# unslothai/unsloth

Hardware: AMD Instinct MI355X
Metric: train tokens/sec, Llama-3-8B QLoRA (NF4) r=16 seq2048 bf16 (higher is better)
Workload: dtype bf16; 1 GPU; Llama-3-8B QLoRA NF4 r=16 (q,k,v,o,gate,up,down) seq2048 bf16, fwd+bwd+AdamW; model=Llama-3-8B (synthetic weights), global_batch=4, seq_len=2048, parallelism=dp1, layers=32, lora_rank=16, gradient_checkpointing=unsloth, gc_schedule_chosen=all (every layer keeps everything), nf4_decoded_weight_mirrors=off (every NF4 weight is decoded at every use INSIDE the timed step), trainable_params=41943040, attention=csrc/attention.hip (causal GQA flash, fwd+bwd), optimizer=FlatAdamW fp32 on LoRA params

## Files before the change

include/unsloth_amd.h:

```cpp
#ifndef UNSLOTH_AMD_H
#define UNSLOTH_AMD_H

#include <stdint.h>

#ifdef __cplusplus
extern "C" {
#endif

#define UAMD_OK 0
#define UAMD_ERR_DTYPE (-1)
#define UAMD_ERR_ARG (-2)
#define UAMD_ERR_ALIGN (-3)

#define UAMD_F32 0
#define UAMD_F16 1
#define UAMD_BF16 2

int uamd_version(void);

int uamd_rms_layernorm_fwd(const void* X, const void* W, void* Y, float* r, int64_t n_rows,
                           int n_cols, int64_t x_row_stride, int64_t y_row_stride, float eps,
                           int gemma, int x_dtype, int w_dtype, void* stream);
int uamd_rms_layernorm_bwd(const void* dY, void* dX, const void* X, const void* W, const float* r,
                           int64_t n_rows, int n_cols, int64_t dy_row_stride,
// ... 124 lines not shown
int uamd_gemm_tn_256(const void* A, int64_t lda, int M, int K, const uamd_gemm_group* groups,
                     int n_groups, int accumulate, int dtype, void* stream);
#define UAMD_TUNE_GLU_VAR 0
#define UAMD_TUNE_GROUP_M 1
#define UAMD_TUNE_STREAM_NT 2
#define UAMD_TUNE_DEQUANT_T 3
#define UAMD_TUNE_ATTN_VAR 4
#define UAMD_TUNE_RMS_VAR 5
#define UAMD_TUNE_GEMM_HALF 6
#define UAMD_TUNE_GEMM_PERSIST 7
#define UAMD_TUNE_DEQUANT_X4 8
#define UAMD_TUNE_GEMM_PLAIN 9
#define UAMD_TUNE_GLU_XA 10
#define UAMD_TUNE_GEMM_S 11
#define UAMD_TUNE_COUNT 12
int uamd_set_tuning(int knob, int value);
int uamd_gemm_nt_nf4(const void* A, int64_t lda, int M, int K, const uamd_gemm_group* groups,
                     int n_groups, int accumulate, int dtype, void* stream);
int uamd_lora_xa(const void* X, int64_t ldx, const void* A, int64_t lda, float* out,
                 int64_t ld_out, int M, int K, int R, int out_cols, int dtype, void* stream);

typedef struct {
    const float* P;
    const void* Z;
    float* out;
    int64_t ldp, ldz, ldo;
    int N;
    int R;
    int out_nr;
    float scale;
} uamd_lora_tn_problem;
int uamd_lora_tn(const uamd_lora_tn_problem* probs, int n_probs, int M, float* workspace,
                 int64_t workspace_floats, int dtype, void* stream);

int uamd_attn_fwd(const void* Q, const void* K, const void* V, void* O, float* LSE, const int64_t* strides,
                  int B, int T, int Hq, int Hk, int D, int lse_stride, float scale, int causal, const int* lo,
                  int dtype, void* stream);
int uamd_attn_bwd(const void* Q, const void* K, const void* V, const void* O, const void* dO, const float* LSE,
                  void* dQ, void* dK, void* dV, float* Delta, const int64_t* strides, int B, int T, int Hq, int Hk,
                  int D, int lse_stride, float scale, int causal, const int* lo, const int* hi, int dtype,
                  void* stream);
int uamd_attn_fwd_band(const void* Q, const void* K, const void* V, void* O, float* LSE, const int64_t* strides,
                       int B, int T, int Hq, int Hk, int D, int lse_stride, float scale, int causal, const int* lo,
                       const int* hi, int dtype, void* stream);

typedef struct {
    const void* W;
    const uint8_t* absmax_u8;
    const float* absmax_f32;
    const float* code2;
    const float* absmax2;
    void* y;
    const float* lora_t;
    const void* lora_b;
    const void* bias;
    int64_t ldw, ld_lb;
    float offset, lora_scale;
    int N, R, blocksize2, lora_b_f32, y_f32, _pad;
} uamd_gemv_group;
int uamd_gemv(const void* x, int K, const uamd_gemv_group* groups, int n_groups, int nf4, int blocksize, int dtype,
              void* stream);
#define UAMD_GEMV_SYNC_BYTES (8 * 256)
#define UAMD_TAG_STRIDE 1024u
typedef struct {
    int mode, Rt, w_f32, glu;
    const void* x2;
// ... 61 lines not shown
```

unsloth_amd/_lib.py:

```python
import ctypes
import os
from contextlib import nullcontext

import torch

c_void_p, c_int, c_int64, c_float = ctypes.c_void_p, ctypes.c_int, ctypes.c_int64, ctypes.c_float

HERE = os.path.dirname(os.path.abspath(__file__))
LIB_PATH = os.environ.get("UNSLOTH_AMD_LIB") or os.path.join(HERE, "lib", "libunsloth_amd.so")

UAMD_F32, UAMD_F16, UAMD_BF16 = 0, 1, 2
_DTYPE_CODE = {torch.float32: UAMD_F32, torch.float16: UAMD_F16, torch.bfloat16: UAMD_BF16}
_ERR = {-1: "unsupported dtype", -2: "invalid argument", -3: "pointer/stride not 16-byte aligned"}


class GemmGroup(ctypes.Structure):

    _fields_ = [
        ("B", c_void_p), ("C", c_void_p), ("absmax", c_void_p), ("lora_xa", c_void_p),
        ("lora_b", c_void_p), ("ldb", c_int64), ("ldc", c_int64), ("ld_xa", c_int64),
        ("ld_lb", c_int64), ("N", c_int), ("R", c_int), ("lora_scale", c_float), ("_pad", c_int),
        ("lora_xk", c_void_p), ("lora_bk", c_void_p), ("ld_xk", c_int64), ("ld_bk", c_int64), ("Rk", c_int),
        ("_pad2", c_int), ("bias", c_void_p),
    ]
# ... 77 lines not shown
    "uamd_gemm_nn_256": (c_int, [c_void_p, c_int64, c_int, c_int, ctypes.POINTER(GemmGroup), c_int, c_int,
                                 c_int, c_void_p]),
    "uamd_gemm_tn_256": (c_int, [c_void_p, c_int64, c_int, c_int, ctypes.POINTER(GemmGroup), c_int, c_int,
                                 c_int, c_void_p]),
    "uamd_set_tuning": (c_int, [c_int, c_int]),
    "uamd_gemm_nt_nf4": (c_int, [c_void_p, c_int64, c_int, c_int, ctypes.POINTER(GemmGroup), c_int,
                                 c_int, c_int, c_void_p]),
    "uamd_lora_xa": (c_int, [c_void_p, c_int64, c_void_p, c_int64, c_void_p, c_int64, c_int, c_int,
                             c_int, c_int, c_int, c_void_p]),
    "uamd_lora_xa2": (c_int, [c_void_p, c_int64, c_void_p, c_int64, c_void_p, c_int64, c_int, c_int,
                              c_int, c_int, c_int, c_void_p]),
    "uamd_lora_xa2k": (c_int, [c_void_p, c_int64, c_void_p, c_int64, c_void_p, c_int64, c_void_p, c_int64, c_int,
                               c_int, c_int, c_int, c_int, c_int, c_void_p]),
    "uamd_add_rms_layernorm_fwd": (c_int, [c_void_p] * 6 + [c_int64, c_int, c_int64, c_int64, c_int64, c_int64, c_float,
                                                             c_int, c_int, c_void_p]),
    "uamd_add_rms_layernorm_bwd": (c_int, [c_void_p] * 6 + [c_int64, c_int, c_int64, c_int64, c_int64, c_int64, c_int,
                                                             c_int, c_void_p]),
    "uamd_lora_prepare": (c_int, [c_void_p, c_void_p, c_int, c_int, c_int, c_void_p]),
    "uamd_adamw_flat": (c_int, [c_void_p, c_void_p, c_void_p, c_void_p, c_int64] + [ctypes.c_double] * 8 + [c_int, c_void_p]),
    "uamd_glu_fwd_xa": (c_int, [c_int, c_void_p, c_void_p, c_void_p, c_int, c_int, c_int64, c_void_p, c_int64, c_int,
                                c_void_p, c_int64, c_int, c_void_p, c_int64, c_int, c_int, c_void_p]),
    "uamd_glu_bwd_xa": (c_int, [c_int, c_void_p, c_void_p, c_void_p, c_int, c_int, c_int64]
                        + [c_void_p, c_int64, c_int, c_void_p, c_int64, c_int, c_void_p, c_int64, c_int] * 2
                        + [c_int, c_void_p]),
    "uamd_glu_xa_workspace": (c_int64, [c_int, c_int, c_int, c_int]),
    "uamd_glu_fwd_xa_ws": (c_int, [c_int, c_void_p, c_void_p, c_void_p, c_int, c_int, c_int64, c_void_p, c_int64, c_int,
                                   c_void_p, c_int64, c_int, c_void_p, c_int64, c_int, c_void_p, c_int64, c_void_p, c_int, c_void_p]),
    "uamd_glu_bwd_xa_ws": (c_int, [c_int, c_void_p, c_void_p, c_void_p, c_int, c_int, c_int64]
                           + [c_void_p, c_int64, c_int, c_void_p, c_int64, c_int, c_void_p, c_int64, c_int] * 2
                           + [c_void_p, c_int64, c_void_p, c_int, c_void_p]),
    "uamd_adamw_shard": (c_int, [c_void_p, c_void_p, c_void_p, c_void_p, c_void_p, c_int64] + [ctypes.c_double] * 8
                         + [c_int, c_void_p]),
    "uamd_lora_tn": (c_int, [ctypes.POINTER(LoraTnProblem), c_int, c_int, c_void_p, c_int64, c_int, c_void_p]),
    "uamd_attn_fwd": (c_int, [c_void_p, c_void_p, c_void_p, c_void_p, c_void_p, ctypes.POINTER(c_int64), c_int, c_int,
                              c_int, c_int, c_int, c_int, c_float, c_int, c_void_p, c_int, c_void_p]),
    "uamd_attn_fwd_band": (c_int, [c_void_p, c_void_p, c_void_p, c_void_p, c_void_p, ctypes.POINTER(c_int64), c_int, c_int,
                                   c_int, c_int, c_int, c_int, c_float, c_int, c_void_p, c_void_p, c_int, c_void_p]),
    "uamd_attn_bwd": (c_int, [c_void_p] * 10 + [ctypes.POINTER(c_int64), c_int, c_int, c_int, c_int, c_int, c_int,
                                               c_float, c_int, c_void_p, c_void_p, c_int, c_void_p]),
    "uamd_gemv": (c_int, [c_void_p, c_int, ctypes.POINTER(GemvGroup), c_int, c_int, c_int, c_int, c_void_p]),
    "uamd_gemv_fused": (c_int, [c_void_p, c_int, ctypes.POINTER(GemvGroup), c_int, c_int, c_int, c_int, c_void_p,
                                ctypes.POINTER(GemvPrologue)]),
    "uamd_rope_kv_append": (c_int, [c_void_p, c_int64, c_void_p, c_void_p, c_int64, c_void_p, c_void_p, c_void_p, c_void_p,
                                    c_int64, c_int64, c_int, c_int, c_int, c_int, c_int, c_int, c_void_p]),
    "uamd_attn_decode": (c_int, [c_void_p, c_int64, c_void_p, c_void_p, c_int64, c_int64, c_void_p, c_int, c_void_p,
                                 c_void_p, c_int64, c_int, c_int, c_int, c_int, c_int, c_int, c_int, c_float, c_int,
                                 c_void_p]),
    "uamd_attn_decode_fused": (c_int, [c_void_p, c_int64, c_void_p, c_void_p, c_int64, c_void_p, c_void_p, c_void_p, c_void_p,
                                       c_int64, c_int64, c_void_p, c_void_p, c_void_p, c_int64, c_int, c_int, c_int, c_int,
                                       c_int, c_int, c_int, c_int, c_float, ctypes.c_uint, c_void_p, c_int, c_void_p]),
    "uamd_argmax_f32": (c_int, [c_void_p, c_int, c_int64, c_void_p, c_void_p, c_void_p, c_void_p]),
    "uamd_debug_mfma_probe": (c_int, [c_void_p, c_void_p]),
}

_LIB = None


def lib():
    global _LIB
    if _LIB is None:
        if not os.path.exists(LIB_PATH):
            raise RuntimeError(
                f"unsloth_amd: {LIB_PATH} is missing. Build it with `python -m unsloth_amd._build` "
                "(hipcc, gfx950). There is no CPU / PyTorch fallback for the fused kernels."
            )
        handle = ctypes.CDLL(LIB_PATH)
# ... 47 lines not shown
```

unsloth_amd/csrc/glu.hip:

```cpp
#include "common.h"

namespace {

enum { ACT_SWIGLU = 0, ACT_GEGLU_EXACT = 1, ACT_GEGLU_APPROX = 2 };
#ifndef UAMD_GLU_KNOCK
#define UAMD_GLU_KNOCK 0
#endif

__device__ __forceinline__ float sigmoidf_(float x) { return uamd_sigmoid(x); }

template <int ACT>
__device__ __forceinline__ void act_fwd(float e, float& f) {
    if (ACT == ACT_SWIGLU) {
        f = e * sigmoidf_(e);
    } else if (ACT == ACT_GEGLU_EXACT) {
        f = 0.5f * e * (erff(0.70710678118654752440f * e) + 1.0f);
    } else {
        const float s = 0.7978845608028654f;
        f = 0.5f * e * (tanhf(s * e * (1.0f + 0.044715f * e * e)) + 1.0f);
    }
}

template <int ACT>
__device__ __forceinline__ void act_bwd(float e, float& f, float& dfde) {
// ... 539 lines not shown
    return UAMD_OK;
}

int64_t xa_ws_floats(int M, int K, int NS, int R) {
    const int NT = R <= 16 ? 1 : (R <= 32 ? 2 : 4);
    const int ntiles = (K + GX_TK - 1) / GX_TK;
    return (int64_t)((M + 15) / 16) * ((ntiles + GX_TPB - 1) / GX_TPB) * 16 * (NS * NT * 16);
}

template <int NS>
int glu_xa_entry(int act, void* dw, void* e, void* g, void* h, int M, int K, int64_t ld, const GluXaOut& o0,
                 const GluXaOut& o1, int dtype, void* stream, float* ws = nullptr, int64_t ws_floats = 0, int* counters = nullptr) {
    if (M < 0 || K <= 0 || !e || !g || (NS == 1 ? !h : !dw)) return UAMD_ERR_ARG;
    if (M == 0) return UAMD_OK;
    if ((K & 7) || (ld & 7) || !aligned16(e) || !aligned16(g) || (NS == 1 ? !aligned16(h) : !aligned16(dw))) return UAMD_ERR_ALIGN;
    int rc = check_xa_out(o0, K);
    if (rc) return rc;
    if (NS > 1 && (rc = check_xa_out(o1, K))) return rc;
    hipStream_t st = (hipStream_t)stream;
    if (ws != nullptr && ws_floats < xa_ws_floats(M, K, NS, NS > 1 ? (o0.R > o1.R ? o0.R : o1.R) : o0.R)) return UAMD_ERR_ARG;
#define GLU_XA_CASE(TT, DC)                                                                          \
    if (dtype == DC) {                                                                              \
        if (act == ACT_SWIGLU) return launch_xa<TT, ACT_SWIGLU, NS>(dw, e, g, h, M, K, ld, o0, o1, st, ws, counters);          \
        if (act == ACT_GEGLU_EXACT) return launch_xa<TT, ACT_GEGLU_EXACT, NS>(dw, e, g, h, M, K, ld, o0, o1, st, ws, counters); \
        if (act == ACT_GEGLU_APPROX) return launch_xa<TT, ACT_GEGLU_APPROX, NS>(dw, e, g, h, M, K, ld, o0, o1, st, ws, counters); \
        return UAMD_ERR_ARG;                                                                        \
    }
    GLU_XA_CASE(bf16_t, UAMD_BF16)
    GLU_XA_CASE(f16_t, UAMD_F16)
#undef GLU_XA_CASE
    return UAMD_ERR_DTYPE;
}

}

extern "C" int uamd_glu_fwd_xa(int act, const void* e, const void* g, void* h, int M, int K, int64_t ld, const void* W,
                               int64_t ldw, int R, float* out, int64_t ld_out, int out_cols, void* out_k, int64_t ld_k,
                               int k_cols, int dtype, void* stream) {
    GluXaOut o0{out, ld_out, R, out_cols, out_k, ld_k, k_cols, W, ldw};
    return glu_xa_entry<1>(act, nullptr, const_cast<void*>(e), const_cast<void*>(g), h, M, K, ld, o0, o0, dtype, stream);
}

extern "C" int uamd_glu_bwd_xa(int act, void* DW, void* e, void* g, int M, int K, int64_t ld,
                               const void* Wu, int64_t ldwu, int Ru, float* out_u, int64_t ld_out_u, int out_cols_u,
                               void* out_k_u, int64_t ld_k_u, int k_cols_u,
                               const void* Wg, int64_t ldwg, int Rg, float* out_g, int64_t ld_out_g, int out_cols_g,
                               void* out_k_g, int64_t ld_k_g, int k_cols_g, int dtype, void* stream) {
    GluXaOut o0{out_u, ld_out_u, Ru, out_cols_u, out_k_u, ld_k_u, k_cols_u, Wu, ldwu};
    GluXaOut o1{out_g, ld_out_g, Rg, out_cols_g, out_k_g, ld_k_g, k_cols_g, Wg, ldwg};
    return glu_xa_entry<2>(act, DW, e, g, nullptr, M, K, ld, o0, o1, dtype, stream);
}

extern "C" int64_t uamd_glu_xa_workspace(int M, int K, int n_products, int max_rank) {
    if (M < 0 || K <= 0 || n_products < 1 || n_products > 2 || max_rank < 1 || max_rank > 64) return -1;
    return xa_ws_floats(M, K, n_products, max_rank);
}
extern "C" int uamd_glu_fwd_xa_ws(int act, const void* e, const void* g, void* h, int M, int K, int64_t ld, const void* W,
                                  int64_t ldw, int R, float* out, int64_t ld_out, int out_cols, void* out_k, int64_t ld_k,
                                  int k_cols, float* ws, int64_t ws_floats, int* counters, int dtype, void* stream) {
    GluXaOut o0{out, ld_out, R, out_cols, out_k, ld_k, k_cols, W, ldw};
    return glu_xa_entry<1>(act, nullptr, const_cast<void*>(e), const_cast<void*>(g), h, M, K, ld, o0, o0, dtype, stream, ws,
                           ws_floats, counters);
}
extern "C" int uamd_glu_bwd_xa_ws(int act, void* DW, void* e, void* g, int M, int K, int64_t ld,
                                  const void* Wu, int64_t ldwu, int Ru, float* out_u, int64_t ld_out_u, int out_cols_u,
                                  void* out_k_u, int64_t ld_k_u, int k_cols_u,
                                  const void* Wg, int64_t ldwg, int Rg, float* out_g, int64_t ld_out_g, int out_cols_g,
                                  void* out_k_g, int64_t ld_k_g, int k_cols_g, float* ws, int64_t ws_floats, int* counters,
                                  int dtype, void* stream) {
    GluXaOut o0{out_u, ld_out_u, Ru, out_cols_u, out_k_u, ld_k_u, k_cols_u, Wu, ldwu};
    GluXaOut o1{out_g, ld_out_g, Rg, out_cols_g, out_k_g, ld_k_g, k_cols_g, Wg, ldwg};
    return glu_xa_entry<2>(act, DW, e, g, nullptr, M, K, ld, o0, o1, dtype, stream, ws, ws_floats, counters);
}

namespace {
template <typename T, bool BWD>
__global__ void __launch_bounds__(256) quick_gelu_kernel(const T* __restrict__ X, T* __restrict__ Y, int64_t n) {
    constexpr int VEC = Vec16<T>::N;
    const int64_t nvec = n / VEC;
    for (int64_t i = (int64_t)blockIdx.x * 256 + threadIdx.x; i < nvec; i += (int64_t)gridDim.x * 256) {
        Vec16<T> x = ld16_m(X + i * VEC, 0), y;
        if (BWD) y = ld16_m(Y + i * VEC, 0);
#pragma unroll
        for (int j = 0; j < VEC; ++j) {
            const float v = to_f32(x.e[j]);
            const float sg = uamd_sigmoid(1.702f * v);
            if (BWD) y.e[j] = from_f32<T>(to_f32(y.e[j]) * (sg + 1.702f * v * sg * (1.0f - sg)));
            else y.e[j] = from_f32<T>(v * sg);
        }
        st16_m(Y + i * VEC, y, 0);
    }
    if (blockIdx.x == 0) {
        for (int64_t k = nvec * VEC + threadIdx.x; k < n; k += 256) {
            const float v = to_f32(X[k]);
            const float sg = uamd_sigmoid(1.702f * v);
            Y[k] = from_f32<T>(BWD ? to_f32(Y[k]) * (sg + 1.702f * v * sg * (1.0f - sg)) : v * sg);
        }
    }
}
template <typename T, bool BWD>
int launch_quick_gelu(const void* x, void* y, int64_t n, hipStream_t st) {
    if (!aligned16(x) || !aligned16(y)) return UAMD_ERR_ALIGN;
    const int64_t nvec = n / Vec16<T>::N;
    int64_t blocks = (nvec + 255) / 256;
    if (blocks < 1) blocks = 1;
    if (blocks > 256 * 16) blocks = 256 * 16;
    hipLaunchKernelGGL((quick_gelu_kernel<T, BWD>), dim3((unsigned)blocks), dim3(256), 0, st, (const T*)x, (T*)y, n);
// ... 36 lines not shown
```

unsloth_amd/kernels/fast_lora.py:

```python
import os

import torch

from .utils import _same_rows, alloc_rows, glu_bwd_terms, glu_fwd_xa
from .utils import (
    GRAD_SINKS,
    grad_sink,
    cast_lora,
    get_lora_parameters,
    lora_dx_terms,
    lora_linear_dx,
    lora_linear_forward,
    lora_tn,
    lora_tn_supported,
)
from .swiglu import swiglu_fg_kernel, swiglu_DWf_DW_dfg_kernel
from .geglu import (
    geglu_exact_forward_kernel,
    geglu_exact_backward_kernel,
    geglu_approx_forward_kernel,
    geglu_approx_backward_kernel,
)

try:
# ... 7 lines not shown
def _lora_grads(X2d, dY2d, A, B, s, dtype):
    if A is None:
        return None, None
    At, Bt = cast_lora(A, dtype).t(), cast_lora(B, dtype).t()
    dA_t = torch.empty_like(At)
    dB_t = torch.empty_like(Bt)
    dA_t.addmm_(X2d.t(), dY2d @ Bt.t(), alpha=s, beta=0)
    dB_t.addmm_(At.t() @ X2d.t(), dY2d, alpha=s, beta=0)
    return dA_t.t(), dB_t.t()


def _lora_grads_fused(items):
    probs, slots, targets, sinks = [], [], [], []
    for (X2d, dY2d, A, B, s, XA, P) in items:
        if A is None:
            slots.append(None)
            continue
        r = A.shape[0]
        slots.append(len(probs))
        probs.append((P, X2d, r, False, s))
        probs.append((XA, dY2d, r, True, s))
        for prm in (A, B):
            sink = grad_sink(prm)
            sinks.append((sink, prm))
            targets.append(sink.grad_view(prm) if sink is not None else None)
    outs = lora_tn(probs, targets if any(t is not None for t in targets) else None)
    for sink, prm in sinks:
        if sink is not None:
            sink.ready(prm)
    outs = [None if sk[0] is not None else o for o, sk in zip(outs, sinks)]
    return [(None, None) if k is None else (outs[k], outs[k + 1]) for k in slots]


_ACT_NAMES = {swiglu_fg_kernel: "swiglu", swiglu_DWf_DW_dfg_kernel: "swiglu",
              geglu_exact_forward_kernel: "geglu_exact", geglu_exact_backward_kernel: "geglu_exact",
              geglu_approx_forward_kernel: "geglu_approx", geglu_approx_backward_kernel: "geglu_approx"}


MERGE_GATE_UP = True


def _gate_up(X, gate, up, return_xa=False):
    outs = None
    widths = [(q.shape[0] if q is not None else W.shape[0]) for (W, q, *_rest) in (gate, up)]
    if (MERGE_GATE_UP and X.is_cuda and X.dtype in (torch.bfloat16, torch.float16) and widths[0] == widths[1]
            and widths[0] % 64 == 0 and all(len(p) <= 5 or p[5] is None for p in (gate, up))):
        M = X.numel() // X.shape[-1]
        eg = alloc_rows(M, 2 * widths[0], X.dtype, X.device)
        outs = [eg[:, :widths[0]], eg[:, widths[0]:]]
    return lora_linear_forward(X, [gate, up], outs=outs, return_xa=return_xa)


def mlp_forward(X, gate, up, down, act_fwd):
    (e, g), xa_gu = _gate_up(X, gate, up, return_xa=True)
    act = _ACT_NAMES.get(act_fwd)
    e2, g2 = e.view(-1, e.shape[-1]), g.view(-1, g.shape[-1])
    fused = glu_fwd_xa(act, e2, g2, down) if (act is not None and _same_rows([e2, g2])) else None
    if fused is not None:
        h, pre = fused
        (out,), xa_d = lora_linear_forward(h.view(e.shape), [down], return_xa=True, pre_xa=pre)
    else:
        if not e.is_contiguous():
            e, g = e.contiguous(), g.contiguous()
        h = act_fwd(e, g)
        (out,), xa_d = lora_linear_forward(h, [down], return_xa=True)
    return out, e, g, (xa_gu[0], xa_gu[1], xa_d[0])


def mlp_gate_up_forward(X, gate, up):
    return _gate_up(X, gate, up)


def mlp_backward(dY, X, e, g, xas, gate, up, down, act_bwd, inplace=True):
    xa_g, xa_u, xa_d = xas
    shape = X.shape
    dY = dY.reshape(-1, dY.shape[-1])
    X2 = X.reshape(-1, X.shape[-1])
    e = e.view(-1, e.shape[-1])
    g = g.view(-1, g.shape[-1])
    dtype = X2.dtype
    (p_d,) = lora_dx_terms([dY], [down])
    padded = e.stride(0) != e.shape[1] and _same_rows([e, g])
    DW = lora_linear_dx([dY], [down], terms=[p_d],
                        out=alloc_rows(e.shape[0], e.shape[1], e.dtype, e.device, ld=e.stride(0)) if padded else None)
    act = _ACT_NAMES.get(act_bwd)
    fused = glu_bwd_terms(act, DW, e, g, up, gate) if (act is not None and DW.dim() == 2) else None
    if fused is not None:
        h, df, de, (p_u, p_g) = fused
    else:
        if padded:
            DW, e, g = DW.contiguous(), e.contiguous(), g.contiguous()
        DW, e, g = act_bwd(DW, e, g)
        h, df, de = DW, e, g
        p_u, p_g = lora_dx_terms([df, de], [up, gate])
    if lora_tn_supported([h, dY, X2, df, de]):
        (d_downA, d_downB), (d_upA, d_upB), (d_gateA, d_gateB) = _lora_grads_fused([
            (h, dY, down[2], down[3], down[4], xa_d, p_d), (X2, df, up[2], up[3], up[4], xa_u, p_u),
            (X2, de, gate[2], gate[3], gate[4], xa_g, p_g)])
    else:
        d_downA, d_downB = _lora_grads(h, dY, down[2], down[3], down[4], dtype)
        d_upA, d_upB = _lora_grads(X2, df, up[2], up[3], up[4], dtype)
        d_gateA, d_gateB = _lora_grads(X2, de, gate[2], gate[3], gate[4], dtype)
    dX = lora_linear_dx([df, de], [up, gate], out=X2 if (inplace and X2.is_contiguous()) else None, terms=[p_u, p_g])
    return dX.view(shape), (d_gateA, d_gateB, d_upA, d_upB, d_downA, d_downB)


def qkv_forward(X, q, k, v):
    (Q, K, V), xa = lora_linear_forward(X, [q, k, v], return_xa=True)
    return Q, K, V, tuple(xa)


def qkv_backward(dQ, dK, dV, X, xas, q, k, v, inplace=True):
    xa_q, xa_k, xa_v = xas
    shape = X.shape
    dQ = dQ.reshape(-1, dQ.shape[-1])
    dK = dK.reshape(-1, dK.shape[-1])
    dV = dV.reshape(-1, dV.shape[-1])
    X2 = X.reshape(-1, X.shape[-1])
    projs = [q, k, v]
    p_q, p_k, p_v = lora_dx_terms([dQ, dK, dV], projs)
    if lora_tn_supported([X2, dQ, dK, dV]):
        (d_QA, d_QB), (d_KA, d_KB), (d_VA, d_VB) = _lora_grads_fused([
            (X2, dQ, q[2], q[3], q[4], xa_q, p_q), (X2, dK, k[2], k[3], k[4], xa_k, p_k),
            (X2, dV, v[2], v[3], v[4], xa_v, p_v)])
    else:
        d_QA, d_QB = _lora_grads(X2, dQ, q[2], q[3], q[4], X2.dtype)
        d_KA, d_KB = _lora_grads(X2, dK, k[2], k[3], k[4], X2.dtype)
        d_VA, d_VB = _lora_grads(X2, dV, v[2], v[3], v[4], X2.dtype)
# ... 149 lines not shown
```

unsloth_amd/kernels/utils.py:

```python
import ctypes
import os

import torch

from .. import _lib
from .. import nf4 as _nf4
from .._lib import GemmGroup

MAX_FUSED_SIZE = 65536
next_power_of_2 = lambda n: 1 << (max(int(n), 1) - 1).bit_length()

FUSED_NF4 = True
FUSED_NF4_MAX_M = 512
GEMM256_MODE = "auto"
GEMM256_MIN_TILES = 160
LORA_XA_V2 = True


def calculate_settings(n):
    BLOCK_SIZE = next_power_of_2(n)
    num_warps = 4
    if BLOCK_SIZE >= 32768:
        num_warps = 32
    elif BLOCK_SIZE >= 8192:
# ... 827 lines not shown
        counters = torch.zeros(max(groups, ent[1].numel() if ent else 0), dtype=torch.int32, device=t.device)
        ent = _GLU_WS[key] = (part, counters)
    return ent


def glu_fwd_xa(act, e, g, down, n_out_cols_hint=None):
    A = down[2]
    if act != "swiglu" or A is None or not _glu_fusable(e.dtype, [e, g], [A.shape[0]], False):
        return None
    M, K = e.shape
    dtype = e.dtype
    r = A.shape[0]
    W, q = down[0], down[1]
    N = q.shape[0] if q is not None else W.shape[0]
    fused_nf4 = q is not None and FUSED_NF4 and M < FUSED_NF4_MAX_M and q.blocksize == 64 and K % 64 == 0
    want_k = (not fused_nf4) and _use_gemm256(M, K, [N])
    Ac = _cached_cast(A, "rowmajor", dtype, lambda: A.to(dtype).contiguous())
    h = alloc_rows(M, K, dtype, e.device, ld=e.stride(0))
    xa = torch.empty((M, r), dtype=torch.float32, device=e.device)
    xk = torch.empty((M, _rank_width(r)), dtype=dtype, device=e.device) if want_k else None
    with _lib.device_ctx(e):
        part, counters = _glu_workspace(e, 1, r)
        rc = _lib.lib().uamd_glu_fwd_xa_ws(_GLU_ACTS[act], _lib.ptr(e), _lib.ptr(g), _lib.ptr(h), M, K, e.stride(0), _lib.ptr(Ac),
                                           Ac.stride(0), r, _lib.ptr(xa), xa.stride(0), r,
                                           _lib.ptr(xk) if xk is not None else None, xk.stride(0) if xk is not None else 0,
                                           xk.shape[1] if xk is not None else 0, _lib.ptr(part), part.numel(), _lib.ptr(counters),
                                           _lib.dtype_code(dtype), _lib.stream_of(e))
    if rc != 0:
        counters.zero_()
    _lib.check(rc, "uamd_glu_fwd_xa_ws")
    return h, (xa, [(0, r)], xk)


def glu_bwd_terms(act, DW, e, g, up, gate):
    (Au, Bu), (Ag, Bg) = (up[2], up[3]), (gate[2], gate[3])
    if act != "swiglu" or Au is None or Ag is None or not _glu_fusable(e.dtype, [DW, e, g], [Au.shape[0], Ag.shape[0]], True):
        return None
    M, K = e.shape
    dtype = e.dtype
    ru, rg = Au.shape[0], Ag.shape[0]
    Kin = [(p[1].shape[1] if p[1] is not None else p[0].shape[1]) for p in (up, gate)]
    want_k = all(_use_gemm256(M, 64, [k]) for k in Kin)
    But = _cached_cast(Bu, "T", dtype, lambda: Bu.to(dtype).t().contiguous())
    Bgt = _cached_cast(Bg, "T", dtype, lambda: Bg.to(dtype).t().contiguous())
    shared = torch.empty((M, ru + rg), dtype=torch.float32, device=e.device)
    xk = torch.empty((M, _rank_width(ru + rg)), dtype=dtype, device=e.device) if want_k else None
    pu, pg = shared[:, :ru], shared[:, ru:]
    null = None
    with _lib.device_ctx(e):
        part, counters = _glu_workspace(e, 2, max(ru, rg))
        rc = _lib.lib().uamd_glu_bwd_xa_ws(
            _GLU_ACTS[act], _lib.ptr(DW), _lib.ptr(e), _lib.ptr(g), M, K, e.stride(0),
            _lib.ptr(But), But.stride(0), ru, _lib.ptr(pu), shared.stride(0), ru,
            _lib.ptr(xk) if want_k else null, xk.stride(0) if want_k else 0, ru if want_k else 0,
            _lib.ptr(Bgt), Bgt.stride(0), rg, _lib.ptr(pg), shared.stride(0), rg,
            _lib.ptr(xk[:, ru:]) if want_k else null, xk.stride(0) if want_k else 0, (xk.shape[1] - ru) if want_k else 0,
            _lib.ptr(part), part.numel(), _lib.ptr(counters), _lib.dtype_code(dtype), _lib.stream_of(e))
    if rc != 0:
        counters.zero_()
    _lib.check(rc, "uamd_glu_bwd_xa_ws")
    if want_k:
        pu._uamd_xk = (xk, 0)
        pg._uamd_xk = (xk, ru)
    return DW, e, g, [pu, pg]


def dense_dw(dY, X, out=None, accumulate=False):
    dY2d, X2d = _rows2d(dY), _rows2d(X)
    _lib.require_gpu(X2d)
    T, N_out = dY2d.shape
    assert X2d.shape[0] == T and X2d.dtype == dY2d.dtype
    dtype = X2d.dtype
    if dtype not in (torch.bfloat16, torch.float16):
        raise NotImplementedError("the MFMA GEMM path takes bf16/fp16 activations")
    N_in = X2d.shape[1]
    if N_out % 8 or N_in % 8:
        raise NotImplementedError(f"dense_dw: out {N_out} / in {N_in} features must be multiples of 8")
    if T % 64:
        pad = 64 - T % 64
        dY2d = torch.nn.functional.pad(dY2d, (0, 0, 0, pad))
        X2d = torch.nn.functional.pad(X2d, (0, 0, 0, pad))
        T += pad
    if dY2d.stride(1) != 1 or dY2d.stride(0) % 8 or dY2d.data_ptr() % 16:
        dY2d = dY2d.contiguous()
    if X2d.stride(1) != 1 or X2d.stride(0) % 8 or X2d.data_ptr() % 16:
        X2d = X2d.contiguous()
    if out is None:
        out = torch.empty((N_out, N_in), dtype=dtype, device=X2d.device)
        accumulate = False
    assert out.dtype == dtype and tuple(out.shape) == (N_out, N_in) and out.stride(1) == 1
    item = X2d.element_size()
    row_bytes = max(dY2d.stride(0), X2d.stride(0)) * item
    step = T if T * row_bytes < GEMM_SPAN_LIMIT else _chunk_rows(row_bytes, 64)
    with _lib.device_ctx(X2d):
        for t0 in range(0, T, step):
            g = _group(X2d, out, N_in, X2d.stride(0))
            g.B += t0 * X2d.stride(0) * item
# ... 51 lines not shown
```

Measured before the change: 36180 tokens/s.

## Fold LoRA weight-gradient TN GEMMs into fused SwiGLU backward kernel

Adds a new HIP kernel that runs the SwiGLU backward elementwise pass, the rank projections onto the up/gate LoRA B matrices, and three LoRA weight-gradient reductions (down A, up B, gate B) in a single pass over the MLP intermediate tiles. Partial sums go to a workspace and are combined by a second reduce kernel. The intent is to avoid re-reading h, df and de from memory in a separate LoRA TN gradient pass. The remaining gradients (down B, up A, gate A) still go through the existing lora_tn path. This adds workspace traffic for the partials and an extra reduce launch, and per-block register and LDS pressure is higher.

```diff
diff --git a/include/unsloth_amd.h b/include/unsloth_amd.h
--- a/include/unsloth_amd.h
+++ b/include/unsloth_amd.h
@@ -180,6 +180,13 @@
 } uamd_lora_tn_problem;
 int uamd_lora_tn(const uamd_lora_tn_problem* probs, int n_probs, int M, float* workspace,
                  int64_t workspace_floats, int dtype, void* stream);
+int64_t uamd_glu_bwd_tn_workspace(int M, int K, int chunk_rows);
+int uamd_glu_bwd_xa_tn(int act, void* DW, void* e, void* g, int M, int K, int64_t ld,
+                       const void* Wu, int64_t ldwu, int Ru, float* out_u, int64_t ld_out_u, int out_cols_u,
+                       void* out_k_u, int64_t ld_k_u, int k_cols_u,
+                       const void* Wg, int64_t ldwg, int Rg, float* out_g, int64_t ld_out_g, int out_cols_g,
+                       void* out_k_g, int64_t ld_k_g, int k_cols_g, const uamd_lora_tn_problem* tn, int chunk_rows,
+                       float* ws, int64_t ws_floats, int dtype, void* stream);
 
 int uamd_attn_fwd(const void* Q, const void* K, const void* V, void* O, float* LSE, const int64_t* strides,
                   int B, int T, int Hq, int Hk, int D, int lse_stride, float scale, int causal, const int* lo,
diff --git a/unsloth_amd/_lib.py b/unsloth_amd/_lib.py
--- a/unsloth_amd/_lib.py
+++ b/unsloth_amd/_lib.py
@@ -133,6 +133,10 @@
     "uamd_adamw_shard": (c_int, [c_void_p, c_void_p, c_void_p, c_void_p, c_void_p, c_int64] + [ctypes.c_double] * 8
                          + [c_int, c_void_p]),
     "uamd_lora_tn": (c_int, [ctypes.POINTER(LoraTnProblem), c_int, c_int, c_void_p, c_int64, c_int, c_void_p]),
+    "uamd_glu_bwd_tn_workspace": (c_int64, [c_int, c_int, c_int]),
+    "uamd_glu_bwd_xa_tn": (c_int, [c_int, c_void_p, c_void_p, c_void_p, c_int, c_int, c_int64]
+                           + [c_void_p, c_int64, c_int, c_void_p, c_int64, c_int, c_void_p, c_int64, c_int] * 2
+                           + [ctypes.POINTER(LoraTnProblem), c_int, c_void_p, c_int64, c_int, c_void_p]),
     "uamd_attn_fwd": (c_int, [c_void_p, c_void_p, c_void_p, c_void_p, c_void_p, ctypes.POINTER(c_int64), c_int, c_int,
                               c_int, c_int, c_int, c_int, c_float, c_int, c_void_p, c_int, c_void_p]),
     "uamd_attn_fwd_band": (c_int, [c_void_p, c_void_p, c_void_p, c_void_p, c_void_p, ctypes.POINTER(c_int64), c_int, c_int,
diff --git a/unsloth_amd/csrc/glu.hip b/unsloth_amd/csrc/glu.hip
--- a/unsloth_amd/csrc/glu.hip
+++ b/unsloth_amd/csrc/glu.hip
@@ -595,6 +595,228 @@
     return UAMD_ERR_DTYPE;
 }
 
+constexpr int GT_LDS = 2 * 3 * GX_TILE + 2 * GX_TILE;
+
+typedef __attribute__((ext_vector_type(4))) short glu_s16x4_t;
+typedef __attribute__((ext_vector_type(4))) _Float16 glu_f16x4_t;
+typedef __attribute__((address_space(3))) glu_s16x4_t glu_lds_s16x4;
+template <typename T> struct GluMfma16;
+template <> struct GluMfma16<bf16_t> {
+    static __device__ __forceinline__ glu_f32x4_t run(glu_s16x4_t a, glu_s16x4_t b, glu_f32x4_t c) {
+        return __builtin_amdgcn_mfma_f32_16x16x16bf16_1k(a, b, c, 0, 0, 0);
+    }
+};
+template <> struct GluMfma16<f16_t> {
+    static __device__ __forceinline__ glu_f32x4_t run(glu_s16x4_t a, glu_s16x4_t b, glu_f32x4_t c) {
+        union { glu_s16x4_t s; glu_f16x4_t h; } ua, ub;
+        ua.s = a; ub.s = b;
+        return __builtin_amdgcn_mfma_f32_16x16x16f16(ua.h, ub.h, c, 0, 0, 0);
+    }
+};
+
+struct GluTnArgs {
+    uamd_lora_tn_problem p[3];
+    int chunk_rows, nslabs, nchunks;
+    int64_t kpad;
+    float* rp;
+    float* cp;
+};
+
+template <typename T>
+__global__ void __launch_bounds__(512, 4)
+glu_bwd_tn_kernel(T* __restrict__ DW, T* __restrict__ E, T* __restrict__ G, int M, int K, int64_t ld, GluXaOut o0, GluXaOut o1,
+                  GluTnArgs a) {
+    extern __shared__ __attribute__((aligned(16))) unsigned char smem[];
+    typedef typename GluMfma<T>::frag frag_t;
+    const int tid = threadIdx.x, lane = tid & 63;
+    const int wave = __builtin_amdgcn_readfirstlane(tid >> 6);
+    const int l15 = lane & 15, l4 = lane >> 4;
+    const int chunk = (int)(blockIdx.x / (unsigned)a.nslabs);
+    const int slab = (int)(blockIdx.x - (unsigned)chunk * (unsigned)a.nslabs);
+    const int c0 = slab * GX_TK;
+    const int r0 = chunk * a.chunk_rows;
+    const int nt = (min(r0 + a.chunk_rows, M) - r0 + 15) / 16;
+    unsigned char* wl = smem + 2 * 3 * GX_TILE;
+    {
+        const int rk = tid >> 5, cc = (tid & 31) * 8;
+#pragma unroll
+        for (int s = 0; s < 2; ++s) {
+            const GluXaOut& o = s == 0 ? o0 : o1;
+            uint4 v = make_uint4(0, 0, 0, 0);
+            if (c0 + cc + 8 <= K) v = *reinterpret_cast<const uint4*>((const T*)o.W + (int64_t)min(rk, o.R - 1) * o.ldw + c0 + cc);
+            *reinterpret_cast<uint4*>(wl + s * GX_TILE + rk * GX_LD + cc * 2) = v;
+        }
+    }
+    const int srow = 2 * wave + (lane >> 5), scol = (lane & 31) * 8;
+    const int c = c0 + scol;
+    const bool col_ok = c + 8 <= K;
+    const int cc = col_ok ? c : 0;
+    const int cw = wave >= 2 ? wave - 2 : 0;
+    const int cq = cw >> 1;
+    const uamd_lora_tn_problem& pq = cq == 0 ? a.p[0] : (cq == 1 ? a.p[1] : a.p[2]);
+    const float* Pq = pq.P + min(l15, pq.R - 1);
+    const int64_t ldp = pq.ldp;
+    const bool rank_ok = l15 < pq.R;
+    glu_f32x4_t cacc[8];
+#pragma unroll
+    for (int j = 0; j < 8; ++j) cacc[j] = glu_f32x4_t{0.f, 0.f, 0.f, 0.f};
+    struct Regs { Vec16<T> e, g, dw; };
+    Regs A, B;
+    auto load_data = [&](int t, Regs& r) {
+        const int row = min(r0 + 16 * t + srow, M - 1);
+        const int64_t off = (int64_t)row * ld + cc;
+        r.e = ld16_nt(E + off);
+        r.g = ld16_nt(G + off);
+        r.dw = ld16_nt(DW + off);
+        __builtin_amdgcn_sched_barrier(0);
+    };
+    auto tile = [&](int t, Regs& r, Regs& rn, int t_next, auto prefetch) {
+        unsigned char* buf = smem + (t & 1) * 3 * GX_TILE;
+        const int m0 = r0 + 16 * t;
+        float pf[4];
+#pragma unroll
+        for (int j = 0; j < 4; ++j) pf[j] = Pq[(int64_t)min(m0 + 4 * l4 + j, M - 1) * ldp];
+        __builtin_amdgcn_sched_barrier(0);
+        if constexpr (decltype(prefetch)::value) load_data(t_next, rn);
+        Vec16<T> h, df, de;
+#pragma unroll
+        for (int j = 0; j < 8; ++j) bwd_one<T, ACT_SWIGLU>(r.dw.e[j], r.e.e[j], r.g.e[j], h.e[j], df.e[j], de.e[j]);
+        if (col_ok && m0 + srow < M) {
+            const int64_t off = (int64_t)(m0 + srow) * ld + c;
+            st16_nt(DW + off, h);
+            st16_nt(E + off, df);
+            st16_nt(G + off, de);
+        }
+        if (!col_ok) {
+            h.raw = make_uint4(0, 0, 0, 0);
+            df.raw = make_uint4(0, 0, 0, 0);
+            de.raw = make_uint4(0, 0, 0, 0);
+        }
+        unsigned char* dst = buf + srow * GX_LD + scol * 2;
+        *reinterpret_cast<uint4*>(dst) = h.raw;
+        *reinterpret_cast<uint4*>(dst + GX_TILE) = df.raw;
+        *reinterpret_cast<uint4*>(dst + 2 * GX_TILE) = de.raw;
+        asm volatile("s_waitcnt lgkmcnt(0)" ::: "memory");
+        __builtin_amdgcn_s_barrier();
+        asm volatile("" ::: "memory");
+        if (wave < 2) {
+            const unsigned char* za = buf + (1 + wave) * GX_TILE + l15 * GX_LD + l4 * 16;
+            const unsigned char* wb = wl + wave * GX_TILE + l15 * GX_LD + l4 * 16;
+            glu_f32x4_t acc = glu_f32x4_t{0.f, 0.f, 0.f, 0.f};
+#pragma unroll
+            for (int q = 0; q < 8; ++q) {
+                union { uint4 r; frag_t f; } x, w;
+                x.r = *reinterpret_cast<const uint4*>(za + q * 64);
+                w.r = *reinterpret_cast<const uint4*>(wb + q * 64);
+                acc = GluMfma<T>::run(x.f, w.f, acc);
+            }
+#pragma unroll
+            for (int i = 0; i < 4; ++i) {
+                const int row = m0 + 4 * l4 + i;
+                if (row < M) a.rp[(((int64_t)row * a.nslabs + slab) * 2 + wave) * 16 + l15] = acc[i];
+            }
+        } else {
+            union { T e[4]; glu_s16x4_t s; } pa;
+#pragma unroll
+            for (int j = 0; j < 4; ++j) pa.e[j] = from_f32<T>(rank_ok && m0 + 4 * l4 + j < M ? pf[j] : 0.f);
+            const unsigned char* zb = buf + cq * GX_TILE + (4 * l4 + (l15 >> 2)) * GX_LD + (cw & 1) * 256 + (l15 & 3) * 8;
+#pragma unroll
+            for (int j = 0; j < 8; ++j) {
+                const glu_s16x4_t b = __builtin_amdgcn_ds_read_tr16_b64_v4i16((glu_lds_s16x4*)(zb + j * 32));
+                cacc[j] = GluMfma16<T>::run(pa.s, b, cacc[j]);
+            }
+        }
+    };
+    constexpr std::true_type yes{};
+    load_data(0, A);
+    int t = 0;
+    for (; t + 1 < nt; t += 2) {
+        tile(t, A, B, t + 1, yes);
+        tile(t + 1, B, A, t + 2 < nt ? t + 2 : t + 1, yes);
+    }
+    if (t < nt) tile(t, A, B, t, yes);
+    if (wave >= 2) {
+        float* cp = a.cp + ((int64_t)chunk * 3 + cq) * 16 * a.kpad + c0 + (cw & 1) * 128 + l15;
+#pragma unroll
+        for (int j = 0; j < 8; ++j)
+#pragma unroll
+            for (int i = 0; i < 4; ++i) cp[(int64_t)(4 * l4 + i) * a.kpad + j * 16] = cacc[j][i];
+    }
+}
+
+template <typename T>
+__global__ void __launch_bounds__(256)
+glu_bwd_tn_reduce_kernel(int M, int K, GluXaOut o0, GluXaOut o1, GluTnArgs a) {
+    const int y = blockIdx.y;
+    const int64_t idx = (int64_t)blockIdx.x * 256 + threadIdx.x;
+    if (y < 2) {
+        const GluXaOut& o = y == 0 ? o0 : o1;
+        const int wide = o.out_cols > o.k_cols ? o.out_cols : o.k_cols;
+        if (idx >= (int64_t)M * wide) return;
+        const int m = (int)(idx / wide), cl = (int)(idx - (int64_t)m * wide);
+        float v = 0.f;
+        if (cl < o.R) {
+            const float* q = a.rp + ((int64_t)m * a.nslabs * 2 + y) * 16 + cl;
+            for (int s = 0; s < a.nslabs; ++s) v += q[(int64_t)s * 32];
+        }
+        if (cl < o.out_cols) o.out[(int64_t)m * o.ld_out + cl] = v;
+        if (o.out_k != nullptr && cl < o.k_cols) ((T*)o.out_k)[(int64_t)m * o.ld_k + cl] = from_f32<T>(v);
+        return;
+    }
+    const int q = y - 2;
+    const uamd_lora_tn_problem& pr = a.p[q];
+    if (idx >= (int64_t)pr.R * K) return;
+    const int r = (int)(idx / K), n = (int)(idx - (int64_t)r * K);
+    const float* part = a.cp + ((int64_t)q * 16 + r) * a.kpad + n;
+    const int64_t cstride = (int64_t)3 * 16 * a.kpad;
+    float v = 0.f;
+    for (int ch = 0; ch < a.nchunks; ++ch) v += part[(int64_t)ch * cstride];
+    v *= pr.scale;
+    float* o = (pr.out_nr & 1) ? pr.out + (int64_t)n * pr.ldo + r : pr.out + (int64_t)r * pr.ldo + n;
+    *o = (pr.out_nr & 2) ? *o + v : v;
+}
+
+constexpr int GT_CHUNK_ROWS = 512;
+
+int64_t tn_ws_floats(int M, int K, int chunk_rows) {
+    const int64_t nslabs = (K + GX_TK - 1) / GX_TK, nchunks = (M + chunk_rows - 1) / chunk_rows;
+    return (int64_t)M * nslabs * 32 + nchunks * 3 * 16 * nslabs * GX_TK;
+}
+
+template <typename T>
+int launch_bwd_tn(void* dw, void* e, void* g, int M, int K, int64_t ld, const GluXaOut& o0, const GluXaOut& o1, GluTnArgs a,
+                  float* ws, hipStream_t st) {
+    static bool attr_set[64] = {false};
+    int dev = 0;
+    if (hipGetDevice(&dev) != hipSuccess || dev < 0 || dev >= 64) dev = 0;
+    if (!attr_set[dev]) {
+        hipError_t err = hipFuncSetAttribute(reinterpret_cast<const void*>(&glu_bwd_tn_kernel<T>),
+                                             hipFuncAttributeMaxDynamicSharedMemorySize, GT_LDS);
+        if (err != hipSuccess) return (int)err;
+        attr_set[dev] = true;
+    }
+    a.nslabs = (K + GX_TK - 1) / GX_TK;
+    a.nchunks = (M + a.chunk_rows - 1) / a.chunk_rows;
+    a.kpad = (int64_t)a.nslabs * GX_TK;
+    a.rp = ws;
+    a.cp = ws + (int64_t)M * a.nslabs * 32;
+    const int64_t blocks = (int64_t)a.nslabs * a.nchunks;
+    if (blocks > 0x7fffffffLL) return UAMD_ERR_ARG;
+    hipLaunchKernelGGL((glu_bwd_tn_kernel<T>), dim3((unsigned)blocks), dim3(512), GT_LDS, st, (T*)dw, (T*)e, (T*)g, M, K, ld,
+                       o0, o1, a);
+    int rc = uamd_launch_status();
+    if (rc) return rc;
+    int64_t need = (int64_t)16 * K;
+    for (const GluXaOut* o : {&o0, &o1}) {
+        const int64_t w = (int64_t)M * (o->out_cols > o->k_cols ? o->out_cols : o->k_cols);
+        if (w > need) need = w;
+    }
+    const int64_t rblocks = (need + 255) / 256;
+    if (rblocks > 0x7fffffffLL) return UAMD_ERR_ARG;
+    hipLaunchKernelGGL((glu_bwd_tn_reduce_kernel<T>), dim3((unsigned)rblocks, 5), dim3(256), 0, st, M, K, o0, o1, a);
+    return uamd_launch_status();
+}
+
 }
 
 extern "C" int uamd_glu_fwd_xa(int act, const void* e, const void* g, void* h, int M, int K, int64_t ld, const void* W,
@@ -636,6 +858,41 @@
     return glu_xa_entry<2>(act, DW, e, g, nullptr, M, K, ld, o0, o1, dtype, stream, ws, ws_floats, counters);
 }
 
+extern "C" int64_t uamd_glu_bwd_tn_workspace(int M, int K, int chunk_rows) {
+    if (chunk_rows <= 0) chunk_rows = GT_CHUNK_ROWS;
+    if (M < 0 || K <= 0 || (chunk_rows & 15)) return -1;
+    return tn_ws_floats(M, K, chunk_rows);
+}
+extern "C" int uamd_glu_bwd_xa_tn(int act, void* DW, void* e, void* g, int M, int K, int64_t ld,
+                                  const void* Wu, int64_t ldwu, int Ru, float* out_u, int64_t ld_out_u, int out_cols_u,
+                                  void* out_k_u, int64_t ld_k_u, int k_cols_u,
+                                  const void* Wg, int64_t ldwg, int Rg, float* out_g, int64_t ld_out_g, int out_cols_g,
+                                  void* out_k_g, int64_t ld_k_g, int k_cols_g, const uamd_lora_tn_problem* tn, int chunk_rows,
+                                  float* ws, int64_t ws_floats, int dtype, void* stream) {
+    if (chunk_rows <= 0) chunk_rows = GT_CHUNK_ROWS;
+    if (act != ACT_SWIGLU || M < 0 || K <= 0 || !DW || !e || !g || !tn || !ws || (chunk_rows & 15)) return UAMD_ERR_ARG;
+    if (M == 0) return UAMD_OK;
+    if ((K & 7) || (ld & 7) || !aligned16(DW) || !aligned16(e) || !aligned16(g)) return UAMD_ERR_ALIGN;
+    GluXaOut o0{out_u, ld_out_u, Ru, out_cols_u, out_k_u, ld_k_u, k_cols_u, Wu, ldwu};
+    GluXaOut o1{out_g, ld_out_g, Rg, out_cols_g, out_k_g, ld_k_g, k_cols_g, Wg, ldwg};
+    int rc = check_xa_out(o0, K);
+    if (rc || (rc = check_xa_out(o1, K))) return rc;
+    if (Ru > 16 || Rg > 16) return UAMD_ERR_ARG;
+    GluTnArgs a;
+    const void* own[3] = {DW, e, g};
+    for (int i = 0; i < 3; ++i) {
+        const uamd_lora_tn_problem& p = tn[i];
+        if (!p.P || !p.out || p.N != K || p.R < 1 || p.R > 16 || (p.Z && p.Z != own[i])) return UAMD_ERR_ARG;
+        a.p[i] = p;
+    }
+    a.chunk_rows = chunk_rows;
+    if (ws_floats < tn_ws_floats(M, K, chunk_rows)) return UAMD_ERR_ARG;
+    hipStream_t st = (hipStream_t)stream;
+    if (dtype == UAMD_BF16) return launch_bwd_tn<bf16_t>(DW, e, g, M, K, ld, o0, o1, a, ws, st);
+    if (dtype == UAMD_F16) return launch_bwd_tn<f16_t>(DW, e, g, M, K, ld, o0, o1, a, ws, st);
+    return UAMD_ERR_DTYPE;
+}
+
 namespace {
 template <typename T, bool BWD>
 __global__ void __launch_bounds__(256) quick_gelu_kernel(const T* __restrict__ X, T* __restrict__ Y, int64_t n) {
diff --git a/unsloth_amd/kernels/fast_lora.py b/unsloth_amd/kernels/fast_lora.py
--- a/unsloth_amd/kernels/fast_lora.py
+++ b/unsloth_amd/kernels/fast_lora.py
@@ -63,6 +63,17 @@
     return [(None, None) if k is None else (outs[k], outs[k + 1]) for k in slots]
 
 
+def _lora_grads_tn(items):
+    sinks = [grad_sink(prm) for (_P, _Z, prm, _R, _nr, _s) in items]
+    targets = [sk.grad_view(prm) if sk is not None else None for sk, (_P, _Z, prm, _R, _nr, _s) in zip(sinks, items)]
+    outs = lora_tn([(P, Z, R, nr, s) for (P, Z, _prm, R, nr, s) in items],
+                   targets if any(t is not None for t in targets) else None)
+    for sk, (_P, _Z, prm, _R, _nr, _s) in zip(sinks, items):
+        if sk is not None:
+            sk.ready(prm)
+    return [None if sk is not None else o for o, sk in zip(outs, sinks)]
+
+
 _ACT_NAMES = {swiglu_fg_kernel: "swiglu", swiglu_DWf_DW_dfg_kernel: "swiglu",
               geglu_exact_forward_kernel: "geglu_exact", geglu_exact_backward_kernel: "geglu_exact",
               geglu_approx_forward_kernel: "geglu_approx", geglu_approx_backward_kernel: "geglu_approx"}
@@ -115,16 +126,36 @@
     DW = lora_linear_dx([dY], [down], terms=[p_d],
                         out=alloc_rows(e.shape[0], e.shape[1], e.dtype, e.device, ld=e.stride(0)) if padded else None)
     act = _ACT_NAMES.get(act_bwd)
-    fused = glu_bwd_terms(act, DW, e, g, up, gate) if (act is not None and DW.dim() == 2) else None
+    tn_items = None
+    if (all(p[2] is not None for p in (down, up, gate)) and lora_tn_supported([DW, e, g, dY, X2])
+            and (act is not None and DW.dim() == 2)):
+        tn_items = [(p_d, down[2], down[4], False), (xa_u, up[3], up[4], True), (xa_g, gate[3], gate[4], True)]
+    tn = None
+    if tn_items is not None:
+        sinks = [grad_sink(prm) for (_P, prm, _s, _nr) in tn_items]
+        tn = [(P, prm.shape[0] if not nr else prm.shape[1], nr, s, sk.grad_view(prm) if sk is not None else None)
+              for (P, prm, s, nr), sk in zip(tn_items, sinks)]
+    fused = glu_bwd_terms(act, DW, e, g, up, gate, tn=tn) if (act is not None and DW.dim() == 2) else None
+    folded = None
+    if fused is not None and tn is not None and fused[4] is not None:
+        for sk, (_P, prm, _s, _nr) in zip(sinks, tn_items):
+            if sk is not None:
+                sk.ready(prm)
+        folded = [None if sk is not None else o for o, sk in zip(fused[4], sinks)]
     if fused is not None:
-        h, df, de, (p_u, p_g) = fused
+        h, df, de, (p_u, p_g) = fused[:4]
     else:
         if padded:
             DW, e, g = DW.contiguous(), e.contiguous(), g.contiguous()
         DW, e, g = act_bwd(DW, e, g)
         h, df, de = DW, e, g
         p_u, p_g = lora_dx_terms([df, de], [up, gate])
-    if lora_tn_supported([h, dY, X2, df, de]):
+    if folded is not None:
+        d_downA, d_upB, d_gateB = folded
+        d_downB, d_upA, d_gateA = _lora_grads_tn([(xa_d, dY, down[3], down[2].shape[0], True, down[4]),
+                                                  (p_u, X2, up[2], up[2].shape[0], False, up[4]),
+                                                  (p_g, X2, gate[2], gate[2].shape[0], False, gate[4])])
+    elif lora_tn_supported([h, dY, X2, df, de]):
         (d_downA, d_downB), (d_upA, d_upB), (d_gateA, d_gateB) = _lora_grads_fused([
             (h, dY, down[2], down[3], down[4], xa_d, p_d), (X2, df, up[2], up[3], up[4], xa_u, p_u),
             (X2, de, gate[2], gate[3], gate[4], xa_g, p_g)])
diff --git a/unsloth_amd/kernels/utils.py b/unsloth_amd/kernels/utils.py
--- a/unsloth_amd/kernels/utils.py
+++ b/unsloth_amd/kernels/utils.py
@@ -883,10 +883,24 @@
     return h, (xa, [(0, r)], xk)
 
 
-def glu_bwd_terms(act, DW, e, g, up, gate):
+GLU_TN_FUSED = True
+GLU_TN_CHUNK_ROWS = 0
+
+
+def _glu_tn_ok(M, tn, ranks):
+    return (GLU_TN_FUSED and all(0 < r <= 16 for r in ranks) and len(tn) == 3
+            and all(P.dtype == torch.float32 and P.dim() == 2 and P.shape[0] == M and P.stride(1) == 1 and 0 < R <= 16
+                    and P.shape[1] >= R for (P, R, _nr, _s, _t) in tn))
+
+
+def glu_bwd_terms(act, DW, e, g, up, gate, tn=None):
     (Au, Bu), (Ag, Bg) = (up[2], up[3]), (gate[2], gate[3])
     if act != "swiglu" or Au is None or Ag is None or not _glu_fusable(e.dtype, [DW, e, g], [Au.shape[0], Ag.shape[0]], True):
         return None
+    if tn is not None:
+        if _glu_tn_ok(e.shape[0], tn, [Au.shape[0], Ag.shape[0]]):
+            return _glu_bwd_tn(act, DW, e, g, up, gate, tn)
+        return glu_bwd_terms(act, DW, e, g, up, gate) + (None,)
     M, K = e.shape
     dtype = e.dtype
     ru, rg = Au.shape[0], Ag.shape[0]
@@ -914,6 +928,50 @@
         pu._uamd_xk = (xk, 0)
         pg._uamd_xk = (xk, ru)
     return DW, e, g, [pu, pg]
+
+
+def _glu_bwd_tn(act, DW, e, g, up, gate, tn):
+    (Au, Bu), (Ag, Bg) = (up[2], up[3]), (gate[2], gate[3])
+    M, K = e.shape
+    dtype = e.dtype
+    ru, rg = Au.shape[0], Ag.shape[0]
+    Kin = [(p[1].shape[1] if p[1] is not None else p[0].shape[1]) for p in (up, gate)]
+    want_k = all(_use_gemm256(M, 64, [k]) for k in Kin)
+    But = _cached_cast(Bu, "T", dtype, lambda: Bu.to(dtype).t().contiguous())
+    Bgt = _cached_cast(Bg, "T", dtype, lambda: Bg.to(dtype).t().contiguous())
+    shared = torch.empty((M, ru + rg), dtype=torch.float32, device=e.device)
+    xk = torch.empty((M, _rank_width(ru + rg)), dtype=dtype, device=e.device) if want_k else None
+    pu, pg = shared[:, :ru], shared[:, ru:]
+    outs, descs = [], []
+    for (P, R, out_nr, scale, tgt) in tn:
+        shape = (K, R) if out_nr else (R, K)
+        if tgt is not None:
+            assert tgt.dtype == torch.float32 and tgt.is_contiguous() and tgt.device == e.device and tuple(tgt.shape) == shape
+            out = tgt
+        else:
+            out = torch.empty(shape, dtype=torch.float32, device=e.device)
+        outs.append(out)
+        descs.append(_lib.LoraTnProblem(P=P.data_ptr(), Z=None, out=out.data_ptr(), ldp=P.stride(0), ldz=0,
+                                        ldo=(R if out_nr else K), N=K, R=R,
+                                        out_nr=int(bool(out_nr)) | (2 if tgt is not None else 0), scale=float(scale)))
+    arr = (_lib.LoraTnProblem * 3)(*descs)
+    L = _lib.lib()
+    null = None
+    with _lib.device_ctx(e):
+        need = int(L.uamd_glu_bwd_tn_workspace(M, K, GLU_TN_CHUNK_ROWS))
+        ws = _nf4.scratch(e.device, need, torch.float32, slot=42)
+        rc = L.uamd_glu_bwd_xa_tn(
+            _GLU_ACTS[act], _lib.ptr(DW), _lib.ptr(e), _lib.ptr(g), M, K, e.stride(0),
+            _lib.ptr(But), But.stride(0), ru, _lib.ptr(pu), shared.stride(0), ru,
+            _lib.ptr(xk) if want_k else null, xk.stride(0) if want_k else 0, ru if want_k else 0,
+            _lib.ptr(Bgt), Bgt.stride(0), rg, _lib.ptr(pg), shared.stride(0), rg,
+            _lib.ptr(xk[:, ru:]) if want_k else null, xk.stride(0) if want_k else 0, (xk.shape[1] - ru) if want_k else 0,
+            arr, GLU_TN_CHUNK_ROWS, _lib.ptr(ws), need, _lib.dtype_code(dtype), _lib.stream_of(e))
+    _lib.check(rc, "uamd_glu_bwd_xa_tn")
+    if want_k:
+        pu._uamd_xk = (xk, 0)
+        pg._uamd_xk = (xk, ru)
+    return DW, e, g, [pu, pg], outs
 
 
 def dense_dw(dY, X, out=None, accumulate=False):
```

Result: faster. 36610 tokens/s, median of 6 (+1.2%).
